# buq2/camera_calibrator

Measured on AMD Instinct MI355X. Metric: LM residuals/sec (2*N_obs per LM iteration), single-camera intrinsics BA, higher is better.
Workload: dtype f64; 1 GPU; BASELINE.json configs[2]: single-camera intrinsics, 1000 frames x 500 pts per GPU, radial-tangential distortion, Zhang init, reference solver options (calibrator.cpp:314-321); frames_total=1000, points_per_frame=500, observations_total=500000, parallelism=frame-sharded x1, exchange=none

## Files before the change

### camera_calibrator_amd/csrc/cc_common.cpp

```cpp
#include "cc_common.hpp"

#include <algorithm>
#include <cstdio>
#include <cstring>
#include <condition_variable>
#include <mutex>
#include <string>
#include <thread>
#include <vector>

namespace cc {

std::string& last_error() {
  static thread_local std::string s;
  return s;
}

double* last_timing() {
  static thread_local double t[5] = {0, 0, 0, 0, 0};
  return t;
}

int fail(int code, const char* fmt, ...) {
  char buf[4096];
// ... 12 lines not shown
  if (hipGetDeviceCount(&n) != hipSuccess || n <= 0)
    return fail(CC_ERR_NO_DEVICE, "no HIP device available (this library has no CPU fallback)");
  if (device < 0 || device >= n) return fail(CC_ERR_BAD_ARGUMENT, "device %d out of range (0..%d)", device, n - 1);
  bool known;
  {
    std::lock_guard<std::mutex> lk(mu);
    if ((int)is_gfx950.size() < n) is_gfx950.resize((size_t)n, 0);
    known = is_gfx950[(size_t)device] != 0;
  }
  if (!known) {
    hipDeviceProp_t prop;
    CC_HIP(hipGetDeviceProperties(&prop, device));
    if (std::string(prop.gcnArchName).rfind("gfx950", 0) != 0)
      return fail(CC_ERR_NO_DEVICE, "device %d is %s; this library is built for gfx950 only", device, prop.gcnArchName);
    std::lock_guard<std::mutex> lk(mu);
    is_gfx950[(size_t)device] = 1;
  }
  CC_HIP(hipSetDevice(device));
  return CC_OK;
}

namespace {
std::mutex g_cache_mu;
std::vector<void*> g_pinned_free;
std::vector<std::vector<hipStream_t>> g_stream_free;
}

void* pinned_block_get() {
  {
    std::lock_guard<std::mutex> lk(g_cache_mu);
    if (!g_pinned_free.empty()) { void* p = g_pinned_free.back(); g_pinned_free.pop_back(); return p; }
  }
  void* p = nullptr;
  if (hipHostMalloc(&p, 512, hipHostMallocDefault) != hipSuccess) { (void)hipGetLastError(); return nullptr; }
  return p;
}

void pinned_block_put(void* p) {
  if (!p) return;
  std::lock_guard<std::mutex> lk(g_cache_mu);
  g_pinned_free.push_back(p);
}

int stream_get(int device, hipStream_t* out) {
  {
    std::lock_guard<std::mutex> lk(g_cache_mu);
    if ((int)g_stream_free.size() > device && !g_stream_free[(size_t)device].empty()) {
      *out = g_stream_free[(size_t)device].back();
      g_stream_free[(size_t)device].pop_back();
      return CC_OK;
    }
  }
  CC_HIP(hipStreamCreateWithFlags(out, hipStreamNonBlocking));
  return CC_OK;
}

namespace {
struct Scratch { void* p = nullptr; size_t bytes = 0; bool busy = false; };
std::vector<Scratch> g_scratch;
constexpr size_t kScratchKeep = (size_t)64 << 20;
}

int scratch_get(int device, size_t bytes, void** out, bool* cached) {
  *cached = false;
  if (bytes <= kScratchKeep) {
    void* old = nullptr;
    bool grow = false, mine = false;
// ... 481 lines not shown
```

### camera_calibrator_amd/csrc/cc_common.hpp

```cpp
#pragma once
#include <hip/hip_runtime.h>
#include <stdint.h>

#include <cmath>
#include <cstdarg>
#include <cstdio>
#include <functional>
#include <mutex>
#include <string>

#include "../../include/cc_solver.h"

namespace cc {

std::string& last_error();
int fail(int code, const char* fmt, ...);

#define CC_HIP(expr)                                                                         \
  do {                                                                                       \
    hipError_t e_ = (expr);                                                                  \
    if (e_ != hipSuccess)                                                                    \
      return ::cc::fail(CC_ERR_HIP, "%s failed: %s (%s:%d)", #expr, hipGetErrorString(e_),   \
                        __FILE__, __LINE__);                                                 \
  } while (0)

int select_device(int device);

void* pinned_block_get();
void pinned_block_put(void* p);
int zhang_on_device(hipStream_t stream, int64_t F, const int64_t* doff, const float* duv, const float* dxyz,
                    double* dgram, float* dH, float* dK, float* dq, float* dt);
int stream_get(int device, hipStream_t* out);
void stream_put(int device, hipStream_t s);
int arena_get(int device, size_t bytes, void** out, bool* cached);
void arena_put(int device, void* p, bool cached);
void* staging_get(size_t bytes, bool* cached);
int pool_alloc(int device, size_t bytes, void** out, size_t* got);
void pool_free(int device, void* p, size_t bytes);
std::mutex& persist_mutex(int device);
bool persist_test_drop_control(const char* env_name, int* remaining);
bool persist_device_try(int device, int kind);
void persist_device_gave_up(int device, int kind);
void persist_device_completed(int device, int kind);
void rig_release_host_caches();
int parallel_parts(int64_t n, int64_t min_per_part);
void parallel_tasks(int parts, const std::function<void(int)>& fn);
void parallel_ranges(int64_t n, int64_t min_per_part, const std::function<void(int, int64_t, int64_t)>& fn);
void last_call_status_reset();
void last_call_status_record(int form, int reruns, const std::string& note);
void parallel_pool_release();
int parallel_pool_threads();
void staging_put(void* p);
double* last_timing();
int scratch_get(int device, size_t bytes, void** out, bool* cached);
void scratch_put(int device, void* p, size_t bytes, bool cached);

constexpr int kP2pMaxRanks = 8;
constexpr long long kP2pTimeoutTicks = 1000000000LL;

struct P2pDev {
// ... 255 lines not shown
```

### camera_calibrator_amd/csrc/cc_intrinsics.hip

```cpp
#include "cc_common.hpp"
#include "cc_device.hpp"
#include "cc_intrinsics_dev.hpp"
#include "cc_intrinsics_persist.hpp"


#include <algorithm>
#include <chrono>
#include <climits>
#include <cstdlib>
#include <cstring>
#include <vector>

namespace cc {

__global__ __launch_bounds__(kSweepThreads, 4) void k_intr_sweep(IntrDev P, int flags) {
  extern __shared__ __attribute__((aligned(16))) char smem_raw[];
  double* s_stage = reinterpret_cast<double*>(smem_raw);
  double* s_blk = s_stage;
  double* sm = s_stage + 4 * kStageDoublesPerWave;
  const int tid = threadIdx.x, lane = tid & 63, wave = tid >> 6;
  const int T = P.T;
  const int64_t f = (int64_t)blockIdx.x / T;
  const int tile = (int)(blockIdx.x - f * T);
  const bool in_solve = (flags & 1) != 0, restart = (flags & 2) != 0;
// ... 828 lines not shown
      { Probe p(h, CC_K_SOLVE, profile, -1); hipLaunchKernelGGL(k_intr_solve<2>, dim3(1), dim3(kSolveThreads), 0, h->stream, h->d, h->elim_blocks, 0); }
    }
    launch_sweep(h, profile, 1);
    { Probe p(h, CC_K_DECIDE, profile); hipLaunchKernelGGL(k_intr_stats_reduce, dim3(1), dim3(256), 0, h->stream, h->d); }
    { Probe p(h, CC_K_ALLREDUCE, profile); if (int rc = comm_allreduce_sum(h->comm, h->d.vec_decide, 16, h->stream)) return rc; }
    { Probe p(h, CC_K_ELIM, profile); hipLaunchKernelGGL(k_intr_decide_elim<2>, dim3(h->elim_blocks), dim3(256), 0, h->stream, h->d, 0); }
    return 0;
  }
  launch_sweep(h, profile, sweep_flags);
  Probe p(h, CC_K_ELIM, profile);
  if (h->exchange) hipLaunchKernelGGL(k_intr_decide_elim<3>, dim3(h->elim_blocks), dim3(256), 0, h->stream, h->d, pub);
  else hipLaunchKernelGGL(k_intr_decide_elim<0>, dim3(h->elim_blocks), dim3(256), 0, h->stream, h->d, pub);
  return 0;
}

static int flush_reset(cc_intrinsics* h) {
  if (!h->reset_pending) return 0;
  launch_reset(h);
  CC_HIP(hipGetLastError());
  h->reset_pending = false;
  return 0;
}

static int read_ctl(cc_intrinsics* h, LmCtl* c) {
  if (int rc = flush_reset(h)) return rc;
  CC_HIP(hipMemcpyAsync(h->h_ctl, h->d.ctl_next, sizeof(LmCtl), hipMemcpyDeviceToHost, h->stream));
  CC_HIP(hipStreamSynchronize(h->stream));
  *c = *h->h_ctl;
  return 0;
}

static int wait_chunk(cc_intrinsics* h, LmCtl* c) {
  return wait_published(h, nullptr, c, nullptr, "the solver", [=] { return read_ctl(h, c); });
}

}

namespace cc {
int intr_create_impl(cc_intrinsics* h, const int64_t* off, const float* uv, const float* xyz);
static thread_local bool g_create_one_shot = false;
static thread_local bool g_create_no_obs = false;
static thread_local size_t g_create_extra = 0;
struct OneShotCreate {
  OneShotCreate(size_t extra, bool no_obs = false) { g_create_one_shot = true; g_create_extra = extra; g_create_no_obs = no_obs; }
  ~OneShotCreate() { g_create_one_shot = false; g_create_extra = 0; g_create_no_obs = false; }
};
static double ms_since(std::chrono::steady_clock::time_point t0) { return std::chrono::duration<double, std::milli>(std::chrono::steady_clock::now() - t0).count(); }
}

extern "C" {

void cc_intrinsics_destroy(cc_intrinsics* h);

int cc_intrinsics_create(int32_t device, int64_t F, const int64_t* off, const float* uv,
                         const float* xyz, cc_intrinsics** out) {
  using namespace cc;
  if (!out || !off || F <= 0) return fail(CC_ERR_BAD_ARGUMENT, "cc_intrinsics_create: bad arguments");
  if (off[0] != 0) return fail(CC_ERR_BAD_ARGUMENT, "frame_offsets[0] must be 0");
  for (int64_t f = 0; f < F; ++f)
    if (off[f + 1] < off[f]) return fail(CC_ERR_BAD_ARGUMENT, "frame_offsets must be non-decreasing");
  const int64_t N = off[F];
  if (F >= ((int64_t)1 << 28) || N >= ((int64_t)1 << 40))
    return fail(CC_ERR_BAD_ARGUMENT, "cc_intrinsics_create: problem too large (frames < 2^28, observations < 2^40)");
  if (N > 0 && (!uv || !xyz) && !cc::g_create_no_obs) return fail(CC_ERR_BAD_ARGUMENT, "uv/xyz are NULL");
  if (int rc = select_device(device)) return rc;
  cc_intrinsics* h = new cc_intrinsics();
// ... 142 lines not shown
  if (!h->one_shot) CC_HIP(hipStreamSynchronize(h->stream));
  d.uv = reinterpret_cast<const float*>(base + o_uv);
  d.xyz = reinterpret_cast<const float*>(base + o_xyz);
  d.off = reinterpret_cast<const int64_t*>(base + o_off);
  d.intr = reinterpret_cast<double*>(base + o_intr);
  d.pose = reinterpret_cast<double*>(base + o_pose);
  d.blocks = reinterpret_cast<double*>(base + o_blocks);
  d.stats = reinterpret_cast<double*>(base + o_stats);
  d.hd0 = reinterpret_cast<double*>(base + o_hd0);
  d.sp = reinterpret_cast<double*>(base + o_sp);
  d.Y = reinterpret_cast<double*>(base + o_Y);
  d.partial = reinterpret_cast<double*>(base + o_partial);
  d.vec_solve = reinterpret_cast<double*>(base + o_vs);
  d.vec_decide = reinterpret_cast<double*>(base + o_vd);
  d.ds = reinterpret_cast<double*>(base + o_ds);
  d.ss = reinterpret_cast<double*>(base + o_ss);
  d.ctl = reinterpret_cast<LmCtl*>(base + o_ctl);
  d.ctl_next = reinterpret_cast<LmCtl*>(base + o_ctln);
  d.arrive = reinterpret_cast<unsigned*>(base + o_sync);
  d.pub_seq = reinterpret_cast<unsigned long long*>(base + o_sync + 8);
  d.opts = reinterpret_cast<LmOpts*>(base + o_opts);
  d.log = reinterpret_cast<cc_iteration*>(base + o_log);
  h->init_intr = reinterpret_cast<double*>(base + o_iintr);
  h->init_pose = reinterpret_cast<double*>(base + o_ipose);
  d.init_intr = h->init_intr;
  d.init_pose = h->init_pose;
  static_assert(16 + sizeof(LmCtl) <= 192 && sizeof(LmCtl) <= 160 && sizeof(LmOpts) <= 160, "one cached 512-byte pinned block holds all three");
  h->pinned = pinned_block_get();
  if (!h->pinned) return fail(CC_ERR_HIP, "hipHostMalloc failed");
  h->host_pub = reinterpret_cast<volatile unsigned long long*>(h->pinned);
  h->h_ctl = reinterpret_cast<LmCtl*>(static_cast<char*>(h->pinned) + 192);
  h->h_opts = reinterpret_cast<LmOpts*>(static_cast<char*>(h->pinned) + 352);
  h->host_pub[0] = 0ull;
  h->pub_count = 0;
  {
    void* dev_view = nullptr;
    CC_HIP(hipHostGetDevicePointer(&dev_view, h->pinned, 0));
    d.host_pub = reinterpret_cast<unsigned long long*>(dev_view);
  }
  h->pq.sbox = reinterpret_cast<unsigned long long*>(base + o_sbox);
  h->pq.pbox = reinterpret_cast<unsigned long long*>(base + o_pbox);
  h->pq.rbox = reinterpret_cast<unsigned long long*>(base + o_rbox);
  h->pq.xbox = reinterpret_cast<unsigned long long*>(base + o_xbox);
  h->pq.fail = reinterpret_cast<unsigned*>(base + o_pfail);
  h->pq.lbox = reinterpret_cast<unsigned long long*>(base + o_lbox);
  h->pq.G = (int32_t)PG;
  h->pq.teams = p_teams;
  h->p_epoch = 0;
  h->persist_ok = p_teams != 0;
  h->elim_blocks = (int)std::min<int64_t>(kElimMaxBlocks, (F + 15) / 16);
  CC_HIP(hipFuncSetAttribute(reinterpret_cast<const void*>(k_intr_sweep),
                             hipFuncAttributeMaxDynamicSharedMemorySize, kSweepLdsBytes));
  CC_HIP(hipFuncSetAttribute(reinterpret_cast<const void*>(k_intr_sweep_huber),
                             hipFuncAttributeMaxDynamicSharedMemorySize, kSweepLdsBytes));
  CC_HIP(hipFuncSetAttribute(reinterpret_cast<const void*>(k_intr_sweep_fisheye),
                             hipFuncAttributeMaxDynamicSharedMemorySize, kSweepLdsBytes));
  return CC_OK;
}
}

extern "C" {

void cc_intrinsics_destroy(cc_intrinsics* h) {
  if (h) cc::last_call_status_record(h->ran_form >= 0 ? h->ran_form : cc_intrinsics_solver_form(h), h->form_reruns, h->form_note);
  if (!h) return;
  hipSetDevice(h->device);
// ... 234 lines not shown
    return fail(CC_ERR_STATE, "LM loop did not terminate (iter=%d)", r->st.iter);
  return 0;
}

static bool use_persistent(const cc_intrinsics* h, const SolveRun* r) {
  return !h->comm && !r->profile && !h->own_sweep() && (h->exchange ? h->persist_x_ok : h->persist_ok);
}

static int persistent_launch(cc_intrinsics* h, SolveRun* r) {
  CC_HIP(hipSetDevice(h->device));
  PersistDev q = h->pq;
  q.max_rounds = r->o.max_iterations + 2;
  q.restart = h->reset_pending ? 1 : 0;
  const uint32_t need = 3u * (uint32_t)q.max_rounds + 3u;
  if (h->p_epoch > 0xf0000000u - need) {
    CC_HIP(hipMemsetAsync(h->pq.sbox, 0, h->p_box_bytes, h->stream));
    h->p_epoch = 0;
  }
  q.epoch0 = h->p_epoch;
  h->p_epoch += need;
  q.timeout_shift = h->exchange ? 30 : 27;
  q.first_shift = h->exchange ? 30 : 20;
  static int drop_left = -2;
  const bool drop_control = !h->exchange && persist_test_drop_control("CC_INTR_PERSIST_TEST_NO_CONTROL", &drop_left);
  persist_launch(h->d, q, drop_control, h->stream);
  CC_HIP(hipGetLastError());
  h->reset_pending = false;
  r->launched = q.max_rounds;
  return 0;
}

static int persistent_wait(cc_intrinsics* h, SolveRun* r) {
  CC_HIP(hipSetDevice(h->device));
  if (int rc = wait_chunk(h, &r->st)) return rc;
  if (r->st.done && r->st.term == CC_FAILURE_EXCHANGE) {
    CC_HIP(hipMemsetAsync(h->pq.fail, 0, sizeof(unsigned), h->stream));
    (void)hipStreamSynchronize(h->stream);
    const std::string where = h->exchange ? mailbox_describe(&h->mailbox, h->d.rank, h->d.nranks) : std::string();
    return fail(CC_ERR_COMM, "persistent solve: a wait inside the kernel timed out (iteration %d): its %d workgroups were not all "
                "resident, or a peer rank did not post within 10 s. %s", r->st.iter, h->pq.G + 1, where.c_str());
  }
  if (!r->st.done) {
    unsigned failed = 0;
    CC_HIP(hipStreamSynchronize(h->stream));
    CC_HIP(hipMemcpy(&failed, h->pq.fail, sizeof(failed), hipMemcpyDeviceToHost));
    if (failed) {
      CC_HIP(hipMemsetAsync(h->pq.fail, 0, sizeof(unsigned), h->stream));
      return fail(CC_ERR_COMM, "persistent solve: the workers' waits timed out and the control workgroup never ran (%d workgroups not all resident)", h->pq.G + 1);
    }
    return fail(CC_ERR_STATE, "persistent solve ended without a result (iter=%d)", r->st.iter);
  }
  return 0;
}

static int solve_persistent(cc_intrinsics* h, SolveRun* r) {
  std::unique_lock<std::mutex> lk(persist_mutex(h->device), std::defer_lock);
  if (!h->exchange && !h->comm) lk.lock();
  if (int rc = persistent_launch(h, r)) return rc;
  return persistent_wait(h, r);
}

}

extern "C" {

int cc_intrinsics_solve(cc_intrinsics* h, const cc_options* opt, cc_summary* summary) {
  using namespace cc;
  if (!h || !h->have_state) return fail(CC_ERR_STATE, "cc_intrinsics_solve: no state set");
  SolveRun r;
  if (int rc = solve_begin(h, opt, &r)) return rc;
  const bool alone = !h->exchange && !h->comm;
  if (use_persistent(h, &r) && (!alone || persist_device_try(h->device, 0))) {
    const bool was_restart = h->reset_pending;
    PersistProbe probe(h->device, 0, alone);
    const int rc = solve_persistent(h, &r);
    if (rc == CC_OK) { probe.completed(); h->ran_form = h->pq.teams; return finish_summary(h, &r, summary); }
    probe.gave_up();
    if (rc != CC_ERR_COMM || h->exchange) return rc;
    h->persist_ok = false;
    h->form_reruns++;
    h->form_note = last_error() + "; the solve was run again with two kernels per iteration and the handle stays on that form";
    CC_HIP(hipStreamSynchronize(h->stream));
    CC_HIP(hipMemsetAsync(h->pq.fail, 0, sizeof(unsigned), h->stream));
    if (was_restart) {
      h->reset_pending = true;
    } else {
      LmCtl zero{};
      if (int rc2 = write_ctl(h, zero)) return rc2;
      CC_HIP(hipMemsetAsync(h->d.arrive, 0, sizeof(unsigned), h->stream));
    }
    h->ctl_fresh = true;
    if (int rc2 = solve_begin(h, opt, &r)) return rc2;
  }
  for (int chunk = 0;; ++chunk) {
    if (int rc = solve_launch(h, &r, chunk)) return rc;
    if (int rc = solve_wait(h, &r)) return rc;
    if (r.st.done) break;
  }
  h->ran_form = 0;
  return finish_summary(h, &r, summary);
}

int cc_intrinsics_optimize_multi(const cc_options* opt, int32_t n_devices, const int32_t* devices, int64_t F,
                                 const int64_t* off, const float* uv, const float* xyz, double* intr9, uint32_t mask,
                                 double* q, double* t, cc_summary* summary) {
  cc::last_call_status_reset();
  using namespace cc;
  if (n_devices < 1 || !devices || n_devices > kP2pMaxRanks)
    return fail(CC_ERR_BAD_ARGUMENT, "cc_intrinsics_optimize_multi: 1..%d devices", kP2pMaxRanks);
// ... 12 lines not shown
    const int64_t f0 = first[(size_t)r], f1 = first[(size_t)r + 1], o0 = off[f0];
    std::vector<int64_t> so((size_t)(f1 - f0) + 1);
    for (int64_t f = f0; f <= f1; ++f) so[(size_t)(f - f0)] = off[f] - o0;
    rc = cc_intrinsics_create(devices[r], f1 - f0, so.data(), uv ? uv + 2 * o0 : nullptr, xyz ? xyz + 3 * o0 : nullptr, &hs[(size_t)r]);
    if (!rc) rc = cc_intrinsics_set_state(hs[(size_t)r], intr9, mask, q + 4 * f0, t + 3 * f0);
  }
  if (!rc) {
    std::vector<Mailbox*> boxes;
    std::vector<int> devs;
    for (auto* h : hs) { boxes.push_back(&h->mailbox); devs.push_back(h->device); }
    for (int r = 0; r < n && !rc; ++r) { rc = hipSetDevice(hs[(size_t)r]->device) == hipSuccess ? mailbox_alloc(&hs[(size_t)r]->mailbox, kVecSolve, 16) : fail(CC_ERR_HIP, "hipSetDevice failed"); }
    for (int r = 0; r < n && !rc; ++r) {
      cc_intrinsics* h = hs[(size_t)r];
      rc = mailbox_wire_local(&h->mailbox, r, n, boxes.data(), devs.data(), &h->d.x);
      if (!rc) { h->d.rank = r; h->d.nranks = n; h->exchange = true; }
    }
  }
  cc_options o;
  if (opt) o = *opt; else cc_options_init(&o);
  o.use_graph = 0;
  std::vector<SolveRun> runs((size_t)n);
  for (int r = 0; r < n && !rc; ++r) rc = solve_begin(hs[(size_t)r], &o, &runs[(size_t)r]);
  bool all_persist = !rc;
  for (int r = 0; r < n && all_persist; ++r) {
    cc_intrinsics* h = hs[(size_t)r];
    int co = 0;
    for (auto* g : hs) if (g->device == h->device) ++co;
    all_persist = h->persist_ok && (int64_t)(h->pq.G + 1) * co <= h->p_resident && !runs[(size_t)r].profile;
  }
  for (auto* h : hs) if (h) h->persist_x_ok = all_persist;
  if (all_persist) {
    for (int r = 0; r < n && !rc; ++r) rc = persistent_launch(hs[(size_t)r], &runs[(size_t)r]);
    for (int r = 0; r < n && !rc; ++r) rc = persistent_wait(hs[(size_t)r], &runs[(size_t)r]);
  }
  for (int chunk = 0; !rc && !all_persist; ++chunk) {
    for (int r = 0; r < n && !rc; ++r) rc = solve_launch(hs[(size_t)r], &runs[(size_t)r], chunk);
    for (int r = 0; r < n && !rc; ++r) rc = solve_wait(hs[(size_t)r], &runs[(size_t)r]);
    if (rc) break;
    bool all_done = true, any_done = false;
    for (auto& run : runs) { all_done = all_done && run.st.done; any_done = any_done || run.st.done; }
    if (all_done) break;
    if (any_done) rc = fail(CC_ERR_STATE, "cc_intrinsics_optimize_multi: the shards disagree about termination");
  }
  if (!rc) rc = finish_summary(hs[0], &runs[0], summary);
  for (int r = 0; r < n && !rc; ++r) {
    const int64_t f0 = first[(size_t)r];
    rc = cc_intrinsics_get_state(hs[(size_t)r], r == 0 ? intr9 : nullptr, q + 4 * f0, t + 3 * f0);
  }
  const std::string err = rc ? last_error() : std::string();
  cleanup();
  if (rc) last_error() = err;
  return rc;
}

int cc_intrinsics_debug_fetch(cc_intrinsics* h, const char* name, double* out, int64_t n) {
  using namespace cc;
  if (!h || !name || !out || n < 0) return fail(CC_ERR_BAD_ARGUMENT, "cc_intrinsics_debug_fetch: bad arguments");
  const std::string k(name);
  const double* src = nullptr;
  int64_t cap = 0;
  if (k == "vec_solve") { src = h->d.vec_solve; cap = kVecSolve; }
  else if (k == "stats") { src = h->d.stats; cap = h->F * h->d.T * kStatsCols; }
  if (!src || n > cap) return fail(CC_ERR_BAD_ARGUMENT, "cc_intrinsics_debug_fetch: unknown buffer or too long");
  CC_HIP(hipSetDevice(h->device));
  CC_HIP(hipStreamSynchronize(h->stream));
  CC_HIP(hipMemcpy(out, src, (size_t)n * sizeof(double), hipMemcpyDeviceToHost));
  return CC_OK;
}

int cc_intrinsics_solver_form(cc_intrinsics* h) {
  if (!h || h->comm || h->own_sweep()) return 0;
  return (h->exchange ? h->persist_x_ok : h->persist_ok) ? h->pq.teams : 0;
}

int cc_intrinsics_solver_status(cc_intrinsics* h, int32_t* form, int32_t* reruns, char* note, int32_t note_capacity) {
  using namespace cc;
  if (!h) return fail(CC_ERR_BAD_ARGUMENT, "cc_intrinsics_solver_status: NULL handle");
  return solver_status(h, cc_intrinsics_solver_form(h), form, reruns, note, note_capacity);
}

int cc_intrinsics_profile_solve(cc_intrinsics* h, const cc_options* opt, int32_t n, double* avg_launch_ms, int32_t* sweeps_per_launch) {
  using namespace cc;
  if (!h || n < 1 || !avg_launch_ms) return fail(CC_ERR_BAD_ARGUMENT, "cc_intrinsics_profile_solve: bad arguments");
  if (!h->have_state) return fail(CC_ERR_STATE, "cc_intrinsics_profile_solve: no state set");
  if (h->huber_a > 0.0) return fail(CC_ERR_STATE, "cc_intrinsics_profile_solve: the handle has a Huber loss set and solves in the two-kernel form");
  if (h->model != CC_MODEL_RADTAN) return fail(CC_ERR_STATE, "cc_intrinsics_profile_solve: the handle has the fisheye model set and solves in the two-kernel form");
  if (!h->persist_ok || h->comm || h->exchange) return fail(CC_ERR_STATE, "cc_intrinsics_profile_solve: the handle does not use the persistent form on a device of its own");
  CC_HIP(hipSetDevice(h->device));
  hipEvent_t e0, e1;
  CC_HIP(hipEventCreate(&e0));
  CC_HIP(hipEventCreate(&e1));
  double total = 0.0;
  int sweeps = 0, rc = 0;
  for (int i = 0; i <= n && !rc; ++i) {
    SolveRun r;
// ... 344 lines not shown
```

### camera_calibrator_amd/csrc/cc_intrinsics_persist.hip

```cpp
#include "cc_intrinsics_persist.hpp"
#include "cc_persist_dev.hpp"
#include "cc_persist_sum.hpp"

namespace cc {


constexpr int persist_lds_doubles(int teams) { return teams * 4 * kStageDoublesPerWave + teams * 2 * 256 + teams * 192 + 512; }

enum { TM_Y = 0, TM_POSE = 60, TM_SP = 76, TM_STEP = 84, TM_R = 100, TM_T = 109, TM_KC = 112, TM_STEP2 = 122, TM_XN2 = 123,
       TM_QW = 124, TM_STAT = 128  };
enum { WG_INTR = 0 , WG_X = 64 , WG_DS = 66 ,
       WG_SS = 80 , WG_R0 = 96 , WG_OPT = 100 ,
       WG_TAB = 104 ,
       WG_TGI = 416 , WG_TZ = 456  };

static_assert(TM_POSE - TM_Y >= 6 * 10 && TM_SP - TM_POSE >= 2 * 8 && TM_STEP - TM_SP >= 6 && TM_R - TM_STEP >= 15 && TM_T - TM_R >= 9 && TM_KC - TM_T >= 3 &&
              TM_STEP2 - TM_KC >= 9 && TM_QW - TM_XN2 >= 1 && TM_STAT - TM_QW >= 4 && TM_STAT + 4 + 9 <= 192,
              "per-team scratch: Y (6 x 10), two poses, pose scale, step (9 + 6), R, t, intrinsics, scalars, statistics row -- inside the 192 doubles persist_lds_doubles gives a team");
static_assert(WG_X - WG_INTR >= 2 * 16 && WG_DS - WG_X >= 2 && WG_SS - WG_DS >= 9 && WG_R0 - WG_SS >= 9 && WG_OPT - WG_R0 >= 1 && WG_TAB - WG_OPT >= 4 &&
              WG_TZ - WG_TGI >= 80 / 2 && WG_TZ + 80 / 2 <= 512,
              "workgroup scratch: both intrinsics, broadcast (2 + 9), scales, options, tables of the 80-slot row -- inside the 512 doubles of persist_lds_doubles");

template <int NC, int NG, int BATCH = 8>
__device__ __forceinline__ void gather_rows(const u64* box, int G, unsigned tag, int ncols, int maxcol, double* s_part,
                                            double* out, unsigned* fail, int* s_ok, int tshift) {
  const int tid = threadIdx.x, col = tid % NC, grp = tid / NC;
  if (tid == 0) *s_ok = 1;
  __syncthreads();
  if (grp < NG && col < ncols) {
    double acc = 0.0;
    bool good = true;
    const long long t0 = wall_clock64();
    for (int r0 = grp; r0 < G && good; r0 += BATCH * NG) {
      u64 lo[BATCH], hi[BATCH];
// ... 143 lines not shown
  const int tid = threadIdx.x;
  if (tid == 0) *s_ok = 1;
  __syncthreads();
  if (tid < kPartialCols) {
    const u64* p = box + 2 * tid;
    u64 lo, hi;
    bool good = true;
    const long long t0 = wall_clock64();
    for (unsigned spins = 0;; ++spins) {
      lo = ag_ld(p);
      hi = ag_ld(p + 1);
      if ((unsigned)(lo >> 32) == tag && (unsigned)(hi >> 32) == tag) break;
      if ((spins & 63u) == 63u && (timed_out(t0, tshift) || ag_ld32(fail) != 0u)) { good = false; break; }
      __builtin_amdgcn_s_sleep(1);
    }
    out[tid] = ungranule(lo, hi);
    if (!good) *s_ok = 0;
  }
  __syncthreads();
}

template <int THREADS>
__device__ __forceinline__ void persist_control(const IntrDev& P, const PersistDev& Q, double* lds) {
  double* s_part = lds;
  double* sv = lds + 1024;
  double* s_tot = lds + 1152;
  double* s_bc = lds + 1168;
  double* s_intr = lds + 1184;
  double* s_ss = lds + 1216;
  LmCtl* s_ctl = reinterpret_cast<LmCtl*>(lds + 1232);
  LmOpts* s_opts = reinterpret_cast<LmOpts*>(lds + 1252);
  cc_iteration* s_log = reinterpret_cast<cc_iteration*>(lds + 1264);
  int* s_int = reinterpret_cast<int*>(lds + 1296);
  const int tid = threadIdx.x, wave = tid >> 6;
  static_assert(sizeof(cc_iteration) <= 32 * 8, "log record scratch");
  if (tid < (int)(sizeof(LmCtl) / 8)) reinterpret_cast<double*>(s_ctl)[tid] = 0.0;
  if (tid >= 32 && tid < 32 + (int)(sizeof(LmOpts) / 8)) reinterpret_cast<u64*>(s_opts)[tid - 32] = reinterpret_cast<const u64*>(P.opts)[tid - 32];
  if (tid >= 64 && tid < 64 + 32) s_intr[tid - 64] = 0.0;
  __syncthreads();
  if (tid < 9) s_intr[tid] = (Q.restart ? P.init_intr : P.intr)[tid];
  if (tid == 0) s_int[1] = 0;
  __syncthreads();
  const LmOpts& o = *s_opts;
  const uint32_t mask = P.mask;

  for (int round = 0; round < Q.max_rounds; ++round) {
    const unsigned e1 = Q.epoch0 + 3u * (unsigned)round + 1u, e2 = e1 + 1u, e3 = e1 + 2u;
    const bool phase0 = round == 0;
    if (phase0) gather_rows<kPStatCols, THREADS / kPStatCols>(Q.sbox, Q.G, e1, 13, -1, s_part, s_tot, Q.fail, s_int, (phase0 ? Q.first_shift : Q.timeout_shift));
    else gather_stats4<THREADS>(Q.sbox, Q.G, e1, s_part, s_tot, Q.fail, s_int, (phase0 ? Q.first_shift : Q.timeout_shift));
    if (P.x.on) {
      const bool need = phase0 || (s_ctl->cand_pending && s_ctl->step_valid);
      if (need) {
        if (tid >= 13 && tid < 16) s_tot[tid] = 0.0;
        __syncthreads();
        const unsigned long long epoch = P.x.seq[1] + 1ull;
        p2p_post(P.x, 1, epoch, P.rank, P.nranks, s_tot, 16);
        int* s_ok2 = s_int + 4;
        const double a = p2p_collect(P.x, 1, epoch, P.rank, P.nranks, 16, s_ok2);
        if (tid < 16) s_tot[tid] = a;
        if (tid == 0) { P.x.seq[1] = epoch; if (!*s_ok2) s_int[0] = 0; }
        __syncthreads();
      }
    }
    if (tid == 0) {
      LmCtl c = *s_ctl;
      const int len0 = c.log_len, prev_cur = c.cur & 1, was_valid = c.step_valid;
      const double prev_radius = c.radius;
      const double* kc0 = s_intr + (c.cur ? 16 : 0);
      const double* kc1 = s_intr + (c.cur ? 0 : 16);
      if (!s_int[0]) {
// ... 5 lines not shown
        for (int i = 0; i < 9; ++i) {
          const double ki = kc0[i];
          xn2 += ki * ki;
          s_ss[i] = o.jacobi_scaling ? 1.0 / (1.0 + sqrt(s_tot[4 + i])) : 1.0;
        }
        lm_init(c, o, s_tot[ST_COST], sqrt(xn2));
      } else if (c.cand_pending) {
        double step2 = s_tot[ST_STEP2], xn2 = s_tot[ST_XNORM2];
        if (c.step_valid) {
#pragma unroll
          for (int i = 0; i < 9; ++i) {
            const double kc = kc1[i], k0 = kc0[i];
            const double d = kc - k0;
            step2 += d * d;
            xn2 += kc * kc;
          }
        }
        lm_decide(c, o, s_log, s_tot[ST_COST], s_tot[ST_QMODEL], step2, xn2);
      }
      if (!c.done && round + 1 >= Q.max_rounds) { c.done = 1; c.term = CC_NO_CONVERGENCE; }
      *s_ctl = c;
      s_int[1] = c.log_len != len0;
      s_int[2] = phase0 ? (!c.done && c.radius == o.initial_radius)
                        : (was_valid && !c.done && (c.cur & 1) == (prev_cur ^ 1) && c.radius == persist_spec_radius(prev_radius, o.max_radius));
      s_bc[0] = (double)((c.done ? 1 : 0) | ((c.cur & 1) << 3));
      s_bc[1] = c.radius;
#pragma unroll
      for (int i = 0; i < 9; ++i) s_bc[2 + i] = 0.0;
    }
    __syncthreads();
    const bool hit = s_int[2] != 0;
    if (s_ctl->done || !hit) {
      if (tid < 22) ag_st(Q.xbox + tid, granule(e2, s_bc[tid >> 1], tid & 1));
      if (s_ctl->done) {
        if (tid == 0 && s_int[1] && s_ctl->log_len <= P.log_cap) P.log[s_ctl->log_len - 1] = *s_log;
        break;
      }
    }
    const unsigned erow = hit ? e2 : e3;
    gather_totals(Q.lbox, erow, sv, Q.fail, s_int, (phase0 ? Q.first_shift : Q.timeout_shift));
    if (P.x.on) {
      if (tid >= kPartialCols && tid < kVecSolve) sv[tid] = 0.0;
      __syncthreads();
      if (tid == 0) { sv[kPartialCols + P.rank] = sv[PC_GMAXP]; sv[PC_GMAXP] = 0.0; }
      __syncthreads();
      const unsigned long long epoch = P.x.seq[0] + 1ull;
      p2p_post(P.x, 0, epoch, P.rank, P.nranks, sv, kVecSolve);
      int* s_ok2 = s_int + 4;
      const double a = p2p_collect(P.x, 0, epoch, P.rank, P.nranks, kVecSolve, s_ok2);
      if (tid < kVecSolve) sv[tid] = a;
      if (tid == 0) { P.x.seq[0] = epoch; if (!*s_ok2) s_int[0] = 0; }
      __syncthreads();
      if (tid == 0) {
        double g = 0.0;
        for (int r = 0; r < P.nranks && r < 32; ++r) g = fmax(g, sv[kPartialCols + r]);
        sv[PC_GMAXP] = g;
      }
      __syncthreads();
    }
    if (wave == 0) {
      int lane = tid & 63;
      asm volatile("" : "+v"(lane));
      const int cur = s_ctl->cur & 1;
      const double radius = s_ctl->radius;
      const double gl = (lane < 9 && !((mask >> lane) & 1u)) ? fabs(sv[PC_GS + lane]) : sv[PC_GMAXP];
      const double k_l = s_intr[cur * 16 + (lane < 9 ? lane : 8)], ss_l = s_ss[lane < 9 ? lane : 8];
      bool ok = !(sv[PC_FAIL] > 0.0);
      double x[9];
      {
#pragma clang fp contract(off)
// ... 13 lines not shown
          a[k] = v;
        }
        const double b = pin_i ? 0.0 : sv[PC_B + i] * si;
        ok = chol_solve_rows<9>(a, b, x) && ok;
#pragma unroll
        for (int j = 0; j < 9; ++j) ok = ok && isfinite(x[j]);
      }
      const double gmax = row16_max(gl);
      const bool go = s_int[0] && !(gmax <= o.gradient_tolerance) && !(radius < o.min_radius);
      if (lane < 9) {
        double xs = 0.0;
#pragma unroll
        for (int j = 0; j < 9; ++j) xs = lane == j ? x[j] : xs;
        const double ds = go ? -xs : 0.0;
        const double d = ((mask >> lane) & 1u) ? 0.0 : ds * ss_l;
        s_bc[2 + lane] = d;
        s_intr[(cur ^ 1) * 16 + lane] = k_l + d;
      }
      if (lane == 0) {
        s_bc[0] = (double)((go ? 0 : 1) | (go && ok ? 2 : 0) | (hit ? 4 : 0) | (cur << 3));
        s_bc[1] = radius;
        s_bc[12] = gmax;
      }
      wave_lds_fence();
      if (lane < 22) ag_st(Q.xbox + lane, granule(erow, s_bc[lane >> 1], lane & 1));
    }
    if (tid == 0) {
      const double gmax = s_bc[12];
      const bool ok = ((int)s_bc[0] & 2) != 0;
      cc_iteration* e = s_int[1] ? s_log : nullptr;
      if (e && e->accepted) e->gradient_max_norm = gmax;
      if (!s_int[0]) { __hip_atomic_store(Q.fail, 1u, __ATOMIC_RELAXED, __HIP_MEMORY_SCOPE_AGENT); s_ctl->done = 1; s_ctl->term = CC_FAILURE_EXCHANGE; }
      else if (lm_finalize(*s_ctl, o, gmax)) { s_ctl->step_valid = ok ? 1 : 0; s_ctl->cand_pending = 1; }
      if (e && s_ctl->log_len <= P.log_cap) P.log[s_ctl->log_len - 1] = *e;
    }
    __syncthreads();
    if (s_ctl->done) break;
  }
  __syncthreads();
  if (tid < 32 && ag_ld32(Q.fail) == 0u) P.intr[tid] = s_intr[tid];
  if (tid == 0) {
    LmCtl c = *s_ctl;
    if (ag_ld32(Q.fail) != 0u) { c.done = 1; c.term = CC_FAILURE_EXCHANGE; }
    if (!c.done) { c.done = 1; c.term = CC_NO_CONVERGENCE; }
    *P.ctl = c;
    *P.ctl_next = c;
    publish_to_host(P, c);
  }
}

template <int TEAMS>
__global__ __launch_bounds__(TEAMS * 256, TEAMS) void k_intr_persist(IntrDev P, PersistDev Q) {
  constexpr int THREADS = TEAMS * 256;
  extern __shared__ __attribute__((aligned(16))) char smem_raw[];
  double* s_stage = reinterpret_cast<double*>(smem_raw);
  if ((int)blockIdx.x == Q.G) { persist_control<THREADS>(P, Q, s_stage); return; }
  double* s_G = s_stage + TEAMS * 4 * kStageDoublesPerWave;
  double* s_tm = s_G + TEAMS * 2 * 256;
  double* s_wg = s_tm + TEAMS * 192;
#define CC_FRESH_TID(name) int name = tid0; asm volatile("" : "+v"(name))
  const int tid0 = threadIdx.x, wave = __builtin_amdgcn_readfirstlane(tid0 >> 6), team = wave >> 2, twave = wave & 3;
  const int sbase = (team & 3) * 64;
  const int64_t f = (int64_t)blockIdx.x * TEAMS + team;
  const bool has_frame = f < P.F;
  double* sm = s_tm + team * 192;
  double* tstage = s_stage + team * 4 * kStageDoublesPerWave;
  double* s_blk = tstage;
  double* Zs = tstage + 1024;
  double* red = tstage + 1100;
  unsigned char* pj = reinterpret_cast<unsigned char*>(s_wg + WG_TAB);
  unsigned char* pk = pj + 48;
  const uint32_t mask = P.mask;

  {
  const int tid = tid0, ttid = tid0 & 255;
  if (has_frame && ttid < 8) {
    const double v = ttid < 7 ? (Q.restart ? P.init_pose : P.pose)[(size_t)f * 8 + ttid] : 0.0;
    sm[TM_POSE + ttid] = v;
    sm[TM_POSE + 8 + ttid] = v;
  }
  if (ttid >= 64 && ttid < 64 + 60) sm[TM_Y + ttid - 64] = 0.0;
// ... 389 lines not shown
```

### camera_calibrator_amd/csrc/cc_solve_host.hpp

```cpp
#pragma once
#include <algorithm>
#include <chrono>
#include <cstring>
#include <string>
#include <vector>

#include "cc_common.hpp"

namespace cc {

struct Comm;
int comm_create(const uint8_t id[128], int rank, int nranks, Comm** out);
void comm_destroy(Comm* c);
int comm_allreduce_sum(Comm* c, double* buf, int n, hipStream_t stream);

struct SolveHost {
  int device = 0;
  hipStream_t stream = nullptr;
  void* pinned = nullptr;
  volatile unsigned long long* host_pub = nullptr;
  unsigned long long pub_count = 0;
  LmCtl* h_ctl = nullptr;
  LmOpts cached_opts{};
  bool opts_valid = false;
  hipGraphExec_t graph[3] = {nullptr, nullptr, nullptr};
  int graph_iters = 0;
  Comm* comm = nullptr;
  Mailbox mailbox;
  bool exchange = false;
  std::vector<hipEvent_t> events;
  std::vector<int> event_kind;
  std::vector<int> event_round;
  int enq_round = 0;
  int ran_form = -1;
  int form_reruns = 0;
  std::string form_note;
};

struct SolveRunBase {
  cc_options o;
// ... 34 lines not shown
  void gave_up() { if (open) persist_device_gave_up(device, kind); open = false; }
  ~PersistProbe() { gave_up(); }
};

template <class H>
static int write_ctl(H* h, const LmCtl& c) {
  CC_HIP(hipMemcpyAsync(h->d.ctl, &c, sizeof(c), hipMemcpyHostToDevice, h->stream));
  CC_HIP(hipMemcpyAsync(h->d.ctl_next, &c, sizeof(c), hipMemcpyHostToDevice, h->stream));
  return 0;
}

template <class ReadCtl>
static int wait_published(SolveHost* h, hipStream_t stream2, LmCtl* c, bool* wait_failed, const char* who, ReadCtl read_ctl) {
  const unsigned long long* word = const_cast<const unsigned long long*>(h->host_pub);
  const unsigned long long want = ++h->pub_count;
  for (unsigned spins = 0;; ++spins) {
    if (__atomic_load_n(word, __ATOMIC_ACQUIRE) == want) break;
    if ((spins & 0xfffu) == 0xfffu) {
      hipError_t q = hipStreamQuery(h->stream);
      if (q == hipSuccess && stream2) q = hipStreamQuery(stream2);
      if (q == hipSuccess) {
        if (__atomic_load_n(word, __ATOMIC_ACQUIRE) == want) break;
        h->pub_count = __atomic_load_n(word, __ATOMIC_ACQUIRE);
        return read_ctl();
      }
      if (q != hipErrorNotReady) return fail(CC_ERR_HIP, "stream failed while waiting for %s: %s", who, hipGetErrorString(q));
    }
  }
  std::memcpy(c, word + 2, sizeof(LmCtl));
  if (wait_failed) *wait_failed = h->host_pub[2 + sizeof(LmCtl) / 8] != 0ull;
  return 0;
}

template <class Enqueue>
static int capture_graph(SolveHost* h, hipGraphExec_t* out, Enqueue enqueue) {
  hipGraph_t g = nullptr;
  CC_HIP(hipStreamBeginCapture(h->stream, hipStreamCaptureModeThreadLocal));
  const int rc = enqueue();
  const hipError_t e_end = hipStreamEndCapture(h->stream, &g);
  if (rc || e_end != hipSuccess) {
    if (g) hipGraphDestroy(g);
    (void)hipGetLastError();
    return rc ? rc : fail(CC_ERR_HIP, "hipStreamEndCapture failed: %s", hipGetErrorString(e_end));
  }
  const hipError_t e_inst = hipGraphInstantiate(out, g, nullptr, nullptr, 0);
  hipGraphDestroy(g);
  if (e_inst != hipSuccess) { *out = nullptr; return fail(CC_ERR_HIP, "hipGraphInstantiate failed: %s", hipGetErrorString(e_inst)); }
  return 0;
}

static int begin_common(SolveHost* h, const cc_options* opt, int log_cap, SolveRunBase* r) {
  r->t0 = std::chrono::steady_clock::now();
  if (opt) r->o = *opt; else cc_options_init(&r->o);
  cc_options& o = r->o;
  if (o.check_interval < 1) o.check_interval = 1;
  if (o.max_iterations > log_cap - 1) o.max_iterations = log_cap - 1;
  r->profile = o.profile_kernels != 0;
  r->use_graph = o.use_graph && !r->profile && !h->comm;
  r->launched = 0;
  CC_HIP(hipSetDevice(h->device));
  clear_probes(h);
  if (r->use_graph && h->graph_iters != o.check_interval) { drop_graphs(h); h->graph_iters = o.check_interval; }
  return 0;
}

static bool opts_changed(SolveHost* h, const LmOpts& lo) {
// ... 49 lines not shown
```

Before: 32.88 billion residuals/s.

## Publish final LM control block as tagged words so host skips fence wait

```diff
diff --git a/camera_calibrator_amd/csrc/cc_common.cpp b/camera_calibrator_amd/csrc/cc_common.cpp
--- a/camera_calibrator_amd/csrc/cc_common.cpp
+++ b/camera_calibrator_amd/csrc/cc_common.cpp
@@ -68,7 +68,7 @@
     if (!g_pinned_free.empty()) { void* p = g_pinned_free.back(); g_pinned_free.pop_back(); return p; }
   }
   void* p = nullptr;
-  if (hipHostMalloc(&p, 512, hipHostMallocDefault) != hipSuccess) { (void)hipGetLastError(); return nullptr; }
+  if (hipHostMalloc(&p, kPinnedBlockBytes, hipHostMallocDefault) != hipSuccess) { (void)hipGetLastError(); return nullptr; }
   return p;
 }
 
diff --git a/camera_calibrator_amd/csrc/cc_common.hpp b/camera_calibrator_amd/csrc/cc_common.hpp
--- a/camera_calibrator_amd/csrc/cc_common.hpp
+++ b/camera_calibrator_amd/csrc/cc_common.hpp
@@ -26,6 +26,7 @@
 
 int select_device(int device);
 
+constexpr size_t kPinnedBlockBytes = 1024;
 void* pinned_block_get();
 void pinned_block_put(void* p);
 int zhang_on_device(hipStream_t stream, int64_t F, const int64_t* doff, const float* duv, const float* dxyz,
diff --git a/camera_calibrator_amd/csrc/cc_intrinsics.hip b/camera_calibrator_amd/csrc/cc_intrinsics.hip
--- a/camera_calibrator_amd/csrc/cc_intrinsics.hip
+++ b/camera_calibrator_amd/csrc/cc_intrinsics.hip
@@ -884,6 +884,10 @@
 
 static int wait_chunk(cc_intrinsics* h, LmCtl* c) {
   return wait_published(h, nullptr, c, nullptr, "the solver", [=] { return read_ctl(h, c); });
+}
+
+static int wait_solve(cc_intrinsics* h, LmCtl* c) {
+  return wait_published_tagged(h, c, "the solver", [=] { return read_ctl(h, c); });
 }
 
 }
@@ -1092,6 +1096,8 @@
   h->h_ctl = reinterpret_cast<LmCtl*>(static_cast<char*>(h->pinned) + 192);
   h->h_opts = reinterpret_cast<LmOpts*>(static_cast<char*>(h->pinned) + 352);
   h->host_pub[0] = 0ull;
+  static_assert((kPubTaggedAt + kPubWords) * 8 <= (int)kPinnedBlockBytes && kPubTaggedAt * 8 >= 512, "the tagged publication lies behind the three blocks");
+  for (int i = 0; i < kPubWords; ++i) h->host_pub[kPubTaggedAt + i] = 0ull;
   h->pub_count = 0;
   {
     void* dev_view = nullptr;
@@ -1392,7 +1398,7 @@
 
 static int persistent_wait(cc_intrinsics* h, SolveRun* r) {
   CC_HIP(hipSetDevice(h->device));
-  if (int rc = wait_chunk(h, &r->st)) return rc;
+  if (int rc = wait_solve(h, &r->st)) return rc;
   if (r->st.done && r->st.term == CC_FAILURE_EXCHANGE) {
     CC_HIP(hipMemsetAsync(h->pq.fail, 0, sizeof(unsigned), h->stream));
     (void)hipStreamSynchronize(h->stream);
@@ -1410,6 +1416,11 @@
     }
     return fail(CC_ERR_STATE, "persistent solve ended without a result (iter=%d)", r->st.iter);
   }
+  return 0;
+}
+
+static int persistent_log_settled(cc_intrinsics* h, const cc_summary* summary) {
+  if (summary && summary->log && summary->log_capacity > 0) CC_HIP(hipStreamSynchronize(h->stream));
   return 0;
 }
 
@@ -1434,7 +1445,12 @@
     const bool was_restart = h->reset_pending;
     PersistProbe probe(h->device, 0, alone);
     const int rc = solve_persistent(h, &r);
-    if (rc == CC_OK) { probe.completed(); h->ran_form = h->pq.teams; return finish_summary(h, &r, summary); }
+    if (rc == CC_OK) {
+      probe.completed();
+      h->ran_form = h->pq.teams;
+      if (int rc2 = persistent_log_settled(h, summary)) return rc2;
+      return finish_summary(h, &r, summary);
+    }
     probe.gave_up();
     if (rc != CC_ERR_COMM || h->exchange) return rc;
     h->persist_ok = false;
@@ -1513,6 +1529,7 @@
   if (all_persist) {
     for (int r = 0; r < n && !rc; ++r) rc = persistent_launch(hs[(size_t)r], &runs[(size_t)r]);
     for (int r = 0; r < n && !rc; ++r) rc = persistent_wait(hs[(size_t)r], &runs[(size_t)r]);
+    if (!rc) rc = persistent_log_settled(hs[0], summary);
   }
   for (int chunk = 0; !rc && !all_persist; ++chunk) {
     for (int r = 0; r < n && !rc; ++r) rc = solve_launch(hs[(size_t)r], &runs[(size_t)r], chunk);
@@ -1542,6 +1559,7 @@
   int64_t cap = 0;
   if (k == "vec_solve") { src = h->d.vec_solve; cap = kVecSolve; }
   else if (k == "stats") { src = h->d.stats; cap = h->F * h->d.T * kStatsCols; }
+  else if (k == "ctl") { src = reinterpret_cast<const double*>(h->d.ctl_next); cap = sizeof(LmCtl) / 8; }
   if (!src || n > cap) return fail(CC_ERR_BAD_ARGUMENT, "cc_intrinsics_debug_fetch: unknown buffer or too long");
   CC_HIP(hipSetDevice(h->device));
   CC_HIP(hipStreamSynchronize(h->stream));
diff --git a/camera_calibrator_amd/csrc/cc_intrinsics_persist.hip b/camera_calibrator_amd/csrc/cc_intrinsics_persist.hip
--- a/camera_calibrator_amd/csrc/cc_intrinsics_persist.hip
+++ b/camera_calibrator_amd/csrc/cc_intrinsics_persist.hip
@@ -1,5 +1,6 @@
 #include "cc_intrinsics_persist.hpp"
 #include "cc_persist_dev.hpp"
+#include "cc_persist_publish.hpp"
 #include "cc_persist_sum.hpp"
 
 namespace cc {
@@ -209,11 +210,13 @@
   LmOpts* s_opts = reinterpret_cast<LmOpts*>(lds + 1252);
   cc_iteration* s_log = reinterpret_cast<cc_iteration*>(lds + 1264);
   int* s_int = reinterpret_cast<int*>(lds + 1296);
+  u64* s_seq = reinterpret_cast<u64*>(lds + 1300);
   const int tid = threadIdx.x, wave = tid >> 6;
   static_assert(sizeof(cc_iteration) <= 32 * 8, "log record scratch");
   if (tid < (int)(sizeof(LmCtl) / 8)) reinterpret_cast<double*>(s_ctl)[tid] = 0.0;
   if (tid >= 32 && tid < 32 + (int)(sizeof(LmOpts) / 8)) reinterpret_cast<u64*>(s_opts)[tid - 32] = reinterpret_cast<const u64*>(P.opts)[tid - 32];
   if (tid >= 64 && tid < 64 + 32) s_intr[tid - 64] = 0.0;
+  if (tid == 48 && P.host_pub) *s_seq = *P.pub_seq + 1ull;
   __syncthreads();
   if (tid < 9) s_intr[tid] = (Q.restart ? P.init_intr : P.intr)[tid];
   if (tid == 0) s_int[1] = 0;
@@ -285,10 +288,7 @@
     const bool hit = s_int[2] != 0;
     if (s_ctl->done || !hit) {
       if (tid < 22) ag_st(Q.xbox + tid, granule(e2, s_bc[tid >> 1], tid & 1));
-      if (s_ctl->done) {
-        if (tid == 0 && s_int[1] && s_ctl->log_len <= P.log_cap) P.log[s_ctl->log_len - 1] = *s_log;
-        break;
-      }
+      if (s_ctl->done) break;
     }
     const unsigned erow = hit ? e2 : e3;
     gather_totals(Q.lbox, erow, sv, Q.fail, s_int, (phase0 ? Q.first_shift : Q.timeout_shift));
@@ -368,21 +368,40 @@
       if (e && e->accepted) e->gradient_max_norm = gmax;
       if (!s_int[0]) { __hip_atomic_store(Q.fail, 1u, __ATOMIC_RELAXED, __HIP_MEMORY_SCOPE_AGENT); s_ctl->done = 1; s_ctl->term = CC_FAILURE_EXCHANGE; }
       else if (lm_finalize(*s_ctl, o, gmax)) { s_ctl->step_valid = ok ? 1 : 0; s_ctl->cand_pending = 1; }
-      if (e && s_ctl->log_len <= P.log_cap) P.log[s_ctl->log_len - 1] = *e;
+      if (e && s_ctl->log_len <= P.log_cap && !s_ctl->done) P.log[s_ctl->log_len - 1] = *e;
     }
     __syncthreads();
     if (s_ctl->done) break;
   }
-  __syncthreads();
-  if (tid < 32 && ag_ld32(Q.fail) == 0u) P.intr[tid] = s_intr[tid];
-  if (tid == 0) {
-    LmCtl c = *s_ctl;
-    if (ag_ld32(Q.fail) != 0u) { c.done = 1; c.term = CC_FAILURE_EXCHANGE; }
-    if (!c.done) { c.done = 1; c.term = CC_NO_CONVERGENCE; }
-    *P.ctl = c;
-    *P.ctl_next = c;
-    publish_to_host(P, c);
-  }
+  if (wave != 0) return;
+  int lane = threadIdx.x;
+  asm volatile("" : "+v"(lane));
+  wave_lds_fence();
+  const unsigned failed = ag_ld32(Q.fail);
+  constexpr int kLogWords = (int)(sizeof(cc_iteration) / 8);
+  static_assert(sizeof(LmCtl) == kPubDoubles * 8 && sizeof(cc_iteration) % 8 == 0 && kLogWords <= 64 && kPubWords <= 64, "one word per lane");
+  static_assert(offsetof(LmCtl, done) == 0 && offsetof(LmCtl, term) == 4, "lanes 0 and 1 hold done and term");
+  unsigned half = reinterpret_cast<const unsigned*>(s_ctl)[lane < kPubWords ? lane : 0];
+  const int done = s_ctl->done, log_len = s_ctl->log_len;
+  const bool owes_record = s_int[1] && log_len <= P.log_cap;
+  const double intr_l = s_intr[lane & 31];
+  const u64 log_l = reinterpret_cast<const u64*>(s_log)[lane < kLogWords ? lane : 0];
+  if (failed != 0u) half = lane == 0 ? 1u : lane == 1 ? (unsigned)CC_FAILURE_EXCHANGE : half;
+  else if (!done) half = lane == 0 ? 1u : lane == 1 ? (unsigned)CC_NO_CONVERGENCE : half;
+  if (P.host_pub) {
+    const u64 seq = *s_seq;
+    if (lane < kPubWords) __hip_atomic_store(P.host_pub + kPubTaggedAt + lane, publish_word(publish_tag(seq), half), __ATOMIC_RELAXED, __HIP_MEMORY_SCOPE_SYSTEM);
+    if (lane == 0) {
+      __hip_atomic_store(P.host_pub, seq, __ATOMIC_RELAXED, __HIP_MEMORY_SCOPE_SYSTEM);
+      *P.pub_seq = seq;
+    }
+  }
+  if (lane < kPubWords) {
+    reinterpret_cast<unsigned*>(P.ctl)[lane] = half;
+    reinterpret_cast<unsigned*>(P.ctl_next)[lane] = half;
+  }
+  if (lane < 32 && failed == 0u) P.intr[lane] = intr_l;
+  if (owes_record && lane < kLogWords) reinterpret_cast<u64*>(P.log + (log_len - 1))[lane] = log_l;
 }
 
 template <int TEAMS>
diff --git a/camera_calibrator_amd/csrc/cc_persist_publish.hpp b/camera_calibrator_amd/csrc/cc_persist_publish.hpp
--- /dev/null
+++ b/camera_calibrator_amd/csrc/cc_persist_publish.hpp
@@ -0,0 +1,36 @@
+#pragma once
+#include <stdint.h>
+
+#ifdef __HIPCC__
+#define CC_PPUB_FN __host__ __device__ __forceinline__
+#else
+#define CC_PPUB_FN inline
+#endif
+
+namespace cc {
+
+constexpr int kPubDoubles = 18;
+constexpr int kPubWords = 2 * kPubDoubles;
+constexpr int kPubTaggedAt = 64;
+
+CC_PPUB_FN uint32_t publish_tag(unsigned long long seq) { return (uint32_t)((seq - 1ull) % 0xffffffffull) + 1u; }
+
+CC_PPUB_FN uint32_t publish_half(unsigned long long bits, int h) { return (uint32_t)(h ? bits >> 32 : bits); }
+
+CC_PPUB_FN unsigned long long publish_word(uint32_t tag, uint32_t half) { return ((unsigned long long)tag << 32) | half; }
+
+CC_PPUB_FN void publish_pack(uint32_t tag, const unsigned long long* block, unsigned long long* tagged) {
+  for (int i = 0; i < kPubWords; ++i) tagged[i] = publish_word(tag, publish_half(block[i >> 1], i & 1));
+}
+
+CC_PPUB_FN bool publish_ready(const unsigned long long* tagged, uint32_t tag) {
+  for (int i = 0; i < kPubWords; ++i)
+    if ((uint32_t)(tagged[i] >> 32) != tag) return false;
+  return true;
+}
+
+CC_PPUB_FN void publish_unpack(const unsigned long long* tagged, unsigned long long* block) {
+  for (int i = 0; i < kPubDoubles; ++i) block[i] = (tagged[2 * i + 1] << 32) | (tagged[2 * i] & 0xffffffffull);
+}
+
+}
diff --git a/camera_calibrator_amd/csrc/cc_solve_host.hpp b/camera_calibrator_amd/csrc/cc_solve_host.hpp
--- a/camera_calibrator_amd/csrc/cc_solve_host.hpp
+++ b/camera_calibrator_amd/csrc/cc_solve_host.hpp
@@ -6,6 +6,7 @@
 #include <vector>
 
 #include "cc_common.hpp"
+#include "cc_persist_publish.hpp"
 
 namespace cc {
 
@@ -106,6 +107,38 @@
   return 0;
 }
 
+template <class ReadCtl>
+static int wait_published_tagged(SolveHost* h, LmCtl* c, const char* who, ReadCtl read_ctl) {
+  static_assert(sizeof(LmCtl) == kPubDoubles * 8, "the tagged publication carries the whole control block");
+  const unsigned long long* word = const_cast<const unsigned long long*>(h->host_pub);
+  const unsigned long long* tagged = word + kPubTaggedAt;
+  const uint32_t want = publish_tag(++h->pub_count);
+  unsigned long long copy[kPubWords];
+  auto arrived = [&] {
+    for (int i = kPubWords - 1; i >= 0; --i) {
+      copy[i] = __atomic_load_n(tagged + i, __ATOMIC_RELAXED);
+      if ((uint32_t)(copy[i] >> 32) != want) return false;
+    }
+    return publish_ready(copy, want);
+  };
+  for (unsigned spins = 0;; ++spins) {
+    if (arrived()) break;
+    if ((spins & 0xfffu) == 0xfffu) {
+      const hipError_t q = hipStreamQuery(h->stream);
+      if (q == hipSuccess) {
+        if (arrived()) break;
+        h->pub_count = __atomic_load_n(word, __ATOMIC_ACQUIRE);
+        return read_ctl();
+      }
+      if (q != hipErrorNotReady) return fail(CC_ERR_HIP, "stream failed while waiting for %s: %s", who, hipGetErrorString(q));
+    }
+  }
+  unsigned long long block[kPubDoubles];
+  publish_unpack(copy, block);
+  std::memcpy(c, block, sizeof(LmCtl));
+  return 0;
+}
+
 template <class Enqueue>
 static int capture_graph(SolveHost* h, hipGraphExec_t* out, Enqueue enqueue) {
   hipGraph_t g = nullptr;
```

Result: no change. 33.27 billion residuals/s (median of 6 runs) (+1.2%).
